# afriesen/rdis

Hardware: AMD Instinct MI355X
Metric: subspace-solver iters/sec (all components), ladybug BA (higher is better)
Workload: dtype f64

## Files before the change

rdis_amd/csrc/minimizer.hpp:

```cpp
#pragma once
#include <hip/hip_runtime.h>
#include <cfloat>
#include <type_traits>
#include <utility>

namespace rdis_hip {

enum : int {
    EXIT_FTOL = 0, EXIT_GTOL = 1, EXIT_GGZERO = 2, EXIT_ITMAX = 3, EXIT_DBRENT_ITMAX = 4,
    EXIT_NAN = 5, EXIT_EMPTY = 6, EXIT_SYNC_TIMEOUT = 7
};
constexpr int STATUS_ROLLED_BACK = 0x100;

enum : int { TR_NONE = 0, TR_F = 1, TR_FD = 2, TR_ITER = 3, TR_START = 4, TR_LINMIN = 5 };

enum : int { REQ_EVAL = 0, REQ_GRAD, REQ_LINE_END, REQ_DONE };
enum : int {
    RF_SLOPE = 1,
    RF_RESTORE = 2,
    RF_LINE = 4,
    RF_PRE_START = 8,
    RF_PRE_UPDATE = 16,
    RF_PRE_BEGIN = 32,
    RF_PRE_LINE_END = 64,
    RF_POST_REDUCE = 128,
    RF_TR_FIRST = 256
};

constexpr int SPEC_MAX = 4;

struct Request {
    int kind;
    int flags;
    int ncand;
    double cand[SPEC_MAX - 1];
    int pre_tag;
    int tr_tag;
    double a, b;
    double pre_a, pre_b, pre_c;
    double tr_a, tr_b, tr_c;
};

__device__ __forceinline__ void opaque(double& v) { asm("" : "+v"(v)); }

struct Predictor {
    enum : int { P_STOP = 0, P_BR_FC, P_DB };
    int ph;
    bool need_first;
    bool known;
    double a, b, x, dx;
    double w, v, dw, dv, d, e;
    double uu;
    double ax, bx, cx;

    __device__ void start(const struct CgdMachine& M, bool swapped);
    __device__ void begin_brent(double ax_, double bx_, double cx_, bool slope_known, double slope) {
        a = (ax_ < cx_ ? ax_ : cx_);
        b = (ax_ > cx_ ? ax_ : cx_);
        x = bx_;
        need_first = !slope_known;
        dx = slope_known ? slope : -1.0;
        ph = P_DB;
        known = false; w = v = x; dw = dv = dx; d = e = 0.0; uu = x;
    }
    __device__ bool next(double& c) {
#pragma clang fp contract(off)
        const double GOLD = 1.618034, TOL = 3.0e-8, ZEPS = DBL_EPSILON * 1.0e-3;
        if (ph == P_BR_FC) {
            cx = bx + GOLD * (bx - ax);
            c = cx;
            if (bx == 0.0) begin_brent(ax, bx, cx, false, 0.0); else ph = P_STOP;
            return true;
        }
        if (ph != P_DB) return false;
        if (need_first) { need_first = false; c = x; return true; }
        const double xm = 0.5 * (a + b);
        const double tol1 = TOL * fabs(x) + ZEPS;
        const double tol2 = 2.0 * tol1;
        if (fabs(x - xm) <= (tol2 - 0.5 * (b - a))) { ph = P_STOP; return false; }
        const double ebis = (dx >= 0.0 ? a - x : b - x);
        const bool near = (uu - x) * (w - x) > 0.0 && fabs(uu - x) < fabs(w - x);
        const bool exact = known && w != x && v != x && v != w && !near;
        double dn = 0.5 * ebis, en = ebis;
        if (exact) {
            const bool big = fabs(e) > tol1;
            const double dflt = 2.0 * (b - a);
            const double q1 = (w - x) * dx / (dx - dw);
            const double q2 = (v - x) * dx / (dx - dv);
            const double d1 = (dw != dx) ? q1 : dflt;
            const double d2 = (dv != dx) ? q2 : dflt;
            const double u1 = x + d1, u2 = x + d2;
            const bool ok1 = (a - u1) * (u1 - b) > 0.0 && dx * d1 <= 0.0;
            const bool ok2 = (a - u2) * (u2 - b) > 0.0 && dx * d2 <= 0.0;
            const double dsel = (ok1 && ok2) ? (fabs(d1) < fabs(d2) ? d1 : d2) : (ok1 ? d1 : d2);
            const bool accept = big && (ok1 || ok2) && (fabs(dsel) <= fabs(0.5 * e));
            const double ut = x + dsel;
            const double dacc = (ut - a < tol2 || b - ut < tol2) ? copysign(tol1, xm - x) : dsel;
            en = accept ? d : ebis;
            dn = accept ? dacc : 0.5 * ebis;
        } else {
            known = false;
        }
        const bool tn = !(fabs(dn) >= tol1);
        const double u = tn ? x + copysign(tol1, dn) : x + dn;
        c = u;
        d = dn; e = en; uu = u;
        if (tn) ph = P_STOP;
        else if (u < x) a = u; else b = u;
// ... 37 lines not shown
    __device__ int status() const { return reason | (rolled_back ? STATUS_ROLLED_BACK : 0); }

    __device__ static Request req(int kind, double a = 0.0, int flags = 0) {
        Request r; r.kind = kind; r.a = a; r.b = 0.0; r.flags = flags;
        r.ncand = 0;
        for (int k = 0; k < SPEC_MAX - 1; ++k) r.cand[k] = 0.0;
        r.pre_tag = TR_NONE; r.pre_a = r.pre_b = r.pre_c = 0.0;
        r.tr_tag = TR_NONE; r.tr_a = r.tr_b = r.tr_c = 0.0;
        return r;
    }
    __device__ Request with_pending(Request r) {
        r.pre_tag = pp_tag; r.pre_a = pp_a; r.pre_b = pp_b; r.pre_c = pp_c;
        pp_tag = TR_NONE;
        return r;
    }
    __device__ static Request traced(Request r, int tag, double ta, double tb, double tc) {
        r.tr_tag = tag; r.tr_a = ta; r.tr_b = tb; r.tr_c = tc;
        return r;
    }
    __device__ Request want_f(double at, bool line = true) { ++nfeval; return req(REQ_EVAL, at, line ? RF_LINE : 0); }
    __device__ Request want_fd(double at, int extra = 0) { ++nfeval; return req(REQ_EVAL, at, RF_SLOPE | RF_LINE | extra); }
    __device__ Request start_line(int pre_ops, double gamma) {
        iter = its;
        ax = 0.0; bx = 1.0;
        fa = fp; sa = 0.0; va = false;
        if (noskip) {
            st = S_BR_FA;
            Request r = want_f(ax);
            r.flags |= pre_ops | RF_PRE_BEGIN;
            r.b = gamma;
            return r;
        }
        ++nfeval;
        pp_tag = TR_F; pp_a = 0.0; pp_b = fp; pp_c = 0.0;
        st = S_BR_FB;
        Request r = with_pending(want_fd(bx, pre_ops | RF_PRE_BEGIN));
        r.b = gamma;
        return r;
    }
    __device__ Request line_done() {
        if (2.0 * fabs(fx - fp) <= ftol * (fabs(fx) + fabs(fp) + 1.0e-18)) {
            st = S_AFTER_LINMIN;
            return traced(req(REQ_LINE_END, x), TR_LINMIN, x, fx, 0.0);
        }
        fret = fx;
        fp = fret;
        ++ngeval;
        st = S_REDUCED;
        Request r = req(REQ_GRAD, x, RF_PRE_LINE_END | RF_POST_REDUCE);
        r.b = fp;
        return traced(r, TR_LINMIN, x, fx, 0.0);
    }

    __device__ __forceinline__ bool hot(double r0, double r1, double& un, int& pre_tag, double& pre_a, double& pre_b,
                                        double& pre_c, Predictor& G) {
#pragma clang fp contract(off)
        const double TOL = 3.0e-8, ZEPS = DBL_EPSILON * 1.0e-3;
        const int DB_ITMAX = 100;
        double a_ = a, b_ = b, x_ = x, w_ = w, v_ = v, fx_ = fx, fw_ = fw, fv_ = fv;
        double dx_ = dx, dw_ = dw, dv_ = dv, d_ = d, e_ = e, uu_ = uu;
        long long nfe_ = nfeval, nge_ = ngeval;
        int ppt_ = pp_tag;
        double ppa_ = pp_a, ppb_ = pp_b, ppc_ = pp_c;
        const bool tiny_ = tiny;
        const int it_ = it;
        if (st != S_DB_EVAL) return false;
        opaque(a_); opaque(b_); opaque(x_); opaque(w_); opaque(v_); opaque(fx_); opaque(fw_); opaque(fv_);
        opaque(dx_); opaque(dw_); opaque(dv_); opaque(d_); opaque(e_); opaque(uu_);
        opaque(ppa_); opaque(ppb_); opaque(ppc_);
        asm("" : "+v"(nfe_), "+v"(nge_), "+v"(ppt_));
        if ((tiny_ && r0 > fx_) || !(it_ + 1 < DB_ITMAX)) return false;
        const double fu = r0, du = r1;
        const bool le = fu <= fx_;
        const bool right = uu_ >= x_, left = uu_ < x_;
        const double a1 = le ? (right ? x_ : a_) : (left ? uu_ : a_);
        const double b1 = le ? (right ? b_ : x_) : (left ? b_ : uu_);
        const bool c1 = !le && (fu <= fw_ || w_ == x_);
        const bool c2 = !le && !c1 && (fu < fv_ || v_ == x_ || v_ == w_);
        const bool vw = le || c1;
        const double v1 = vw ? w_ : (c2 ? uu_ : v_), fv1 = vw ? fw_ : (c2 ? fu : fv_), dv1 = vw ? dw_ : (c2 ? du : dv_);
        const double w1 = le ? x_ : (c1 ? uu_ : w_), fw1 = le ? fx_ : (c1 ? fu : fw_), dw1 = le ? dx_ : (c1 ? du : dw_);
        const double x1 = le ? uu_ : x_, fx1 = le ? fu : fx_, dx1 = le ? du : dx_;
        const double xm = 0.5 * (a1 + b1);
        const double tol1 = TOL * fabs(x1) + ZEPS;
        const double tol2 = 2.0 * tol1;
        if (fabs(x1 - xm) <= (tol2 - 0.5 * (b1 - a1))) return false;
        const bool big = fabs(e_) > tol1;
        const double dflt = 2.0 * (b1 - a1);
        const double q1 = (w1 - x1) * dx1 / (dx1 - dw1);
        const double q2 = (v1 - x1) * dx1 / (dx1 - dv1);
        const double d1 = (dw1 != dx1) ? q1 : dflt;
        const double d2 = (dv1 != dx1) ? q2 : dflt;
        const double u1 = x1 + d1, u2 = x1 + d2;
        const bool ok1 = (a1 - u1) * (u1 - b1) > 0.0 && dx1 * d1 <= 0.0;
        const bool ok2 = (a1 - u2) * (u2 - b1) > 0.0 && dx1 * d2 <= 0.0;
        const double dsel = (ok1 && ok2) ? (fabs(d1) < fabs(d2) ? d1 : d2) : (ok1 ? d1 : d2);
        const bool accept = big && (ok1 || ok2) && (fabs(dsel) <= fabs(0.5 * e_));
        const double ut = x1 + dsel;
        const double dacc = (ut - a1 < tol2 || b1 - ut < tol2) ? copysign(tol1, xm - x1) : dsel;
        const double ebis = (dx1 >= 0.0 ? a1 - x1 : b1 - x1);
        const double enew = accept ? d_ : ebis;
        const double dnew = accept ? dacc : 0.5 * ebis;
        const bool tn = !(fabs(dnew) >= tol1);
        un = tn ? x1 + copysign(tol1, dnew) : x1 + dnew;
        if (fu != fu) saw_nan = true;
        a = a1; b = b1; v = v1; fv = fv1; dv = dv1; w = w1; fw = fw1; dw = dw1; x = x1; fx = fx1; dx = dx1;
        e = enew; d = dnew; tiny = tn; uu = un;
        it = it_ + 1;
        ngeval = nge_ + 1;
        nfeval = nfe_ + 1;
        pp_tag = TR_NONE;
        pre_tag = ppt_; pre_a = ppa_; pre_b = ppb_; pre_c = ppc_;
        G.need_first = false;
        G.a = (!tn && un < x1) ? un : a1;
        G.b = (!tn && !(un < x1)) ? un : b1;
        G.x = x1; G.dx = dx1;
        G.known = true; G.w = w1; G.v = v1; G.dw = dw1; G.dv = dv1; G.d = dnew; G.e = enew; G.uu = un;
        G.ph = tn ? Predictor::P_STOP : Predictor::P_DB;
        return true;
    }

    __device__ Request next(double r0, double r1, double r2) {
#pragma clang fp contract(off)
        const double GOLD = 1.618034, GLIMIT = 100.0, TINY = 1.0e-20;
        const double GTOL = 1.0e-8;
        const double TOL = 3.0e-8;
        const double ZEPS = DBL_EPSILON * 1.0e-3;
        const int DB_ITMAX = 100;
        for (;;) {
            switch (st) {
            case S_BEGIN:
                st = S_FIRST;
                return want_f(0.0, false);
            case S_FIRST:
                finit = r0;
                if (r0 != r0) saw_nan = true;
                ++nfeval;
                fp = finit;
                ++ngeval;
                st = S_GRAD0;
                return traced(req(REQ_GRAD), TR_START, fp, 0.0, 0.0);
            case S_GRAD0:
                its = 0;
                return start_line(RF_PRE_START, 0.0);

            case S_BR_FA:
                fa = r0; if (r0 != r0) saw_nan = true;
                st = S_BR_FB;
                return want_fd(bx);
            case S_BR_FB:
                fb = r0; sb = r1; vb = true; if (r0 != r0) saw_nan = true;
                if (fb > fa) {
                    double t = ax; ax = bx; bx = t; t = fa; fa = fb; fb = t;
                    t = sa; sa = sb; sb = t; const bool tv = va; va = vb; vb = tv;
                }
                cx = bx + GOLD * (bx - ax);
                st = S_BR_FC;
                return want_fd(cx);
            case S_BR_FC:
                fc = r0; sc = r1; vc = true; if (r0 != r0) saw_nan = true;
                st = S_BR_HEAD;
                break;
            case S_BR_HEAD: {
                if (!(fb > fc)) { st = S_DB_START; break; }
                const double r = (bx - ax) * (fb - fc);
                const double q = (bx - cx) * (fb - fa);
                const double qr = q - r;
                u = bx - ((bx - cx) * q - (bx - ax) * r) / (2.0 * copysign(fmax(fabs(qr), TINY), qr));
                const double ulim = bx + GLIMIT * (cx - bx);
                if ((bx - u) * (u - cx) > 0.0) { st = S_BR_CASE1; return want_fd(u); }
                if ((cx - u) * (u - ulim) > 0.0) { st = S_BR_CASE2; return want_fd(u); }
                if ((u - ulim) * (ulim - cx) >= 0.0) u = ulim;
// ... 122 lines not shown
                if (test < GTOL) { reason = EXIT_GTOL; st = S_FINISH; nx = finish_request(); }
                else if (gg == 0.0) { reason = EXIT_GGZERO; st = S_FINISH; nx = finish_request(); }
                else if (its + 1 >= maxiters) { reason = EXIT_ITMAX; st = S_FINISH; nx = finish_request(); }
                else { ++its; nx = start_line(RF_PRE_UPDATE, dgg / gg); nx.flags |= RF_TR_FIRST; }
                return traced(nx, TR_ITER, test, gg, dgg);
            }

            case S_FINISH: {
                Request nx = finish_request();
                return nx;
            }
            case S_ROLLED:
                fret = r0;
                st = S_DONE;
                return req(REQ_DONE);
            default:
                return req(REQ_DONE);
            }
        }
    }

    __device__ Request finish_request() {
        if (saw_nan) { reason = EXIT_NAN; fret = DBL_MAX; }
        if (fret > finit || saw_nan) {
            rolled_back = true;
            st = S_ROLLED;
            Request r = want_f(0.0, false);
            r.flags |= RF_RESTORE;
            return r;
        }
        st = S_DONE;
        return req(REQ_DONE);
    }
};

__device__ inline void Predictor::start(const CgdMachine& M, bool swapped) {
#pragma clang fp contract(off)
    ph = P_STOP; need_first = false; known = false;
    a = b = x = dx = 0.0; ax = bx = cx = 0.0;
    w = v = dw = dv = d = e = uu = 0.0;
    switch (M.st) {
    case CgdMachine::S_BR_FB:
        if (swapped) { ax = M.bx; bx = M.ax; ph = P_BR_FC; }
        else { ax = M.ax; bx = M.bx; ph = P_BR_FC; }
        break;
    case CgdMachine::S_BR_FC:
        begin_brent(M.ax, M.bx, M.cx, M.vb, M.sb);
        break;
    case CgdMachine::S_DB_FIRST:
        a = M.a; b = M.b; x = M.x; dx = -1.0; ph = P_DB;
        w = v = x; dw = dv = dx; uu = x;
        break;
    case CgdMachine::S_DB_EVAL:
        if (M.tiny) break;
        a = M.a; b = M.b; x = M.x; dx = M.dx; ph = P_DB;
        if (M.uu < x) a = M.uu; else b = M.uu;
        known = true; w = M.w; v = M.v; dw = M.dw; dv = M.dv; d = M.d; e = M.e; uu = M.uu;
        break;
    default: break;
    }
}

__device__ __forceinline__ void step_machine(CgdMachine* __restrict__ M, Request* __restrict__ out, double r0, double r1, double r2,
                                             bool writer) {
    double un, pa, pb, pc;
    int ptag;
    Predictor G;
    if (M->hot(r0, r1, un, ptag, pa, pb, pc, G)) {
        if (writer) {
            out->kind = REQ_EVAL; out->flags = RF_SLOPE | RF_LINE; out->ncand = 0;
            out->pre_tag = ptag; out->tr_tag = TR_NONE; out->a = un;
            if (ptag != TR_NONE) { out->pre_a = pa; out->pre_b = pb; out->pre_c = pc; }
        }
        return;
    }
    const Request nq = M->next(r0, r1, r2);
    if (writer) {
        out->kind = nq.kind; out->flags = nq.flags; out->ncand = 0;
        out->pre_tag = nq.pre_tag; out->tr_tag = nq.tr_tag; out->a = nq.a; out->b = nq.b;
        if (nq.pre_tag != TR_NONE) { out->pre_a = nq.pre_a; out->pre_b = nq.pre_b; out->pre_c = nq.pre_c; }
        if (nq.tr_tag != TR_NONE) { out->tr_a = nq.tr_a; out->tr_b = nq.tr_b; out->tr_c = nq.tr_c; }
    }
}

__device__ __forceinline__ double uniform(double v) {
    const long long b = __double_as_longlong(v);
    const unsigned lo = __builtin_amdgcn_readfirstlane((unsigned)b);
    const unsigned hi = __builtin_amdgcn_readfirstlane((unsigned)((unsigned long long)b >> 32));
    return __longlong_as_double((long long)(((unsigned long long)hi << 32) | lo));
}

template <class Env>
__device__ __forceinline__ double uni(double v) {
    if constexpr (Env::UNIFORM) return uniform(v); else return v;
}
template <class Env>
__device__ __forceinline__ int uni(int v) {
    if constexpr (Env::UNIFORM) return __builtin_amdgcn_readfirstlane(v); else return v;
}

template <int N>
__device__ __forceinline__ double pick(const double (&v)[N], int j) {
    double r = v[0];
#pragma unroll
    for (int k = 1; k < N; ++k) r = (j == k) ? v[k] : r;
    return r;
}
__device__ __forceinline__ bool same_bits(double a, double b) { return __double_as_longlong(a) == __double_as_longlong(b); }

template <class E, class = void> struct EnvNoSkip { static constexpr bool value = false; };
// ... 178 lines not shown
```

rdis_amd/csrc/solver_pipe.hpp:

```cpp
#pragma once
#include "solver_coop.hpp"

namespace rdis_hip {

constexpr int PIPE_NBUF = 32;
constexpr int PIPE_DEPTH = 3;
constexpr int PIPE_ENT = 512;
constexpr int PIPE_MAILS = 4;
constexpr int PIPE_THREADS = 256;
constexpr int PIPE_CTRL = 2;
constexpr int PIPE_LANES = PIPE_THREADS - 64 * PIPE_CTRL;
constexpr int PIPE_QUIT = 0x7FFFFFFF;
static_assert(PIPE_NBUF >= 5 * PIPE_DEPTH + 4 && (PIPE_NBUF & (PIPE_NBUF - 1)) == 0, "ring too short for the run-ahead");

struct PipeState {
    alignas(32) unsigned long long granule[2][PIPE_NBUF][PIPE_ENT][2];
    unsigned int abort_flag;
    unsigned int pad[15];
};
static_assert(sizeof(PipeState) <= sizeof(CoopState), "PipeState must fit the exchange state the host allocates");

struct alignas(16) PipeMail {
    int kind, flags;
    int e;
    int pad0;
    double a, b;
    double g_a, g_b, g_x, g_dx, g_ax, g_bx, g_cx;
    int g_need_first, g_known;
    double g_w, g_v, g_dw, g_dv, g_d, g_e, g_uu;
    int g_ph, pad1;
};
static_assert(sizeof(PipeMail) == 160, "mail layout");
constexpr int PIPE_RES = 4;
static_assert(PIPE_RES > PIPE_DEPTH, "result ring");
constexpr int PIPE_RECS = 8;
struct PipeShared {
    PipeMail mail[PIPE_MAILS];
    alignas(8) int seq;
    int verified;
    int pred_seq;
    int rec_slot[PIPE_RECS];
    double rec_val[PIPE_RECS];
    int cmd, cmd_delay;
    int res_slot[PIPE_RES];
    double res[PIPE_RES][3];
    int bar_done;
    int pub[PIPE_LANES / 64];
    int dead;
    int status, rolled_back, iter;
    long long nfeval, ngeval;
    double fret, finit;
};
typedef __attribute__((address_space(3))) int lds_i32;
typedef __attribute__((address_space(3))) double lds_f64;
__device__ __forceinline__ int lds_int(const int& x) { return *(const volatile lds_i32*)&x; }
__device__ __forceinline__ void lds_set(int& x, int v) { *(volatile lds_i32*)&x = v; }
typedef __attribute__((address_space(3))) long long lds_i64;
__device__ __forceinline__ long long lds_int_pair(const int& x) { return *(const volatile lds_i64*)&x; }
__device__ __forceinline__ double lds_f64_get(const double& x) { return *(const volatile lds_f64*)&x; }
__device__ __forceinline__ void lds_f64_set(double& x, double v) { *(volatile lds_f64*)&x = v; }

struct PipeSync {
    PipeState* st;
    int tid, nwg, wg, nw;
    int poll_delay;
    int e;
    int rearmed;
    bool dead;
#ifdef RDIS_COOP_TIMING
    long long tm[COOP_TM];
#endif
    __device__ void tick(int slot, long long dt) {
#ifdef RDIS_COOP_TIMING
        tm[slot] += dt;
#endif
    }
    __device__ gu64* gran(int ex, int k, int w) const { return (gu64*)&st->granule[k >> 1][ex & (PIPE_NBUF - 1)][w][k & 1]; }
    __device__ u64x2 load_pair(int ex, int k, int w) const {
        u64x2 r;
        const gu64* p = gran(ex, k, w);
        asm volatile("global_load_dwordx4 %0, %1, off sc1" : "=v"(r) : "v"(p) : "memory");
        return r;
    }
    __device__ void store_pair(int ex, int k, int w, unsigned long long a, unsigned long long b) const {
        u64x2 t; t.x = a; t.y = b;
        gu64* p = gran(ex, k, w);
        asm volatile("global_store_dwordx4 %0, %1, off sc1" : : "v"(p), "v"(t) : "memory");
    }

    template <int N, int NMAX>
    __device__ void publish(int ex, double (&v)[N], int* pub) {
#pragma unroll
        for (int k = 0; k < N; ++k) v[k] = k < N - NMAX ? wave_sum(v[k]) : wave_max(v[k]);
        asm volatile("s_waitcnt vmcnt(0)" ::: "memory");
        if ((tid & 63) == 0) {
            const int ent = wg * nw + (tid >> 6) - PIPE_CTRL;
#pragma unroll
            for (int k = 0; k + 1 < N; k += 2) store_pair(ex, k, ent, GridSync::bits_of(v[k]), GridSync::bits_of(v[k + 1]));
            if constexpr (N & 1) GridSync::publish(gran(ex, N - 1, ent), v[N - 1]);
            lds_set(pub[(tid >> 6) - PIPE_CTRL], ex);
        }
    }

    template <int N, int NMAX>
// ... 297 lines not shown
        { const double gn = -wv.xi; const double hn = gn + gam * wv.h; wv.g = gn; wv.h = hn; wv.xi = hn; }
    }
    __device__ void write_back(const VarState& V, bool restore, bool writer) {
        if (V.li >= 0 && writer) {
            const double xf = clampd(restore ? V.xinit : V.p, V.lo, V.hi);
            P.x[L.free_vid[f0 + V.li]] = xf;
            L.xout[f0 + V.li] = xf;
        }
    }
};

__device__ __forceinline__ int pipe_slot_owner(int i) {
    return (i == 0 || i == 2 || i == 3 || i == 18 || (i >= 9 && i <= 11) || i == 30 || i == 31) ? 2 : (i == 1 || (i >= 4 && i <= 6) || (i >= 26 && i <= 29)) ? 1 : 0;
}

__device__ __forceinline__ void pipe_post(PipeShared& S, int seq, int kind, int flags, int e, double a, double b, bool writer) {
    if (writer) {
        PipeMail* m = &S.mail[seq & (PIPE_MAILS - 1)];
        m->kind = kind; m->flags = flags; m->e = e; m->pad0 = 0; m->a = a; m->b = b;
        asm volatile("" ::: "memory");
        lds_set(S.seq, seq);
    }
}
__device__ __forceinline__ void pipe_post_predictor(PipeShared& S, int seq, const Predictor& G, bool writer) {
    if (writer) {
        PipeMail* m = &S.mail[seq & (PIPE_MAILS - 1)];
        m->g_ph = G.ph; m->g_need_first = G.need_first ? 1 : 0; m->g_known = G.known ? 1 : 0; m->pad1 = 0;
        m->g_a = G.a; m->g_b = G.b; m->g_x = G.x; m->g_dx = G.dx; m->g_ax = G.ax; m->g_bx = G.bx; m->g_cx = G.cx;
        m->g_w = G.w; m->g_v = G.v; m->g_dw = G.dw; m->g_dv = G.dv; m->g_d = G.d; m->g_e = G.e; m->g_uu = G.uu;
        asm volatile("" ::: "memory");
        lds_set(S.pred_seq, seq);
    }
}
__device__ __forceinline__ void pipe_command(PipeShared& S, int ex, int n, int delay, bool writer) {
    if (writer) { lds_set(S.cmd_delay, delay); lds_set(S.cmd, (ex << 2) | n); }
}
template <int N>
__device__ __forceinline__ void pipe_result(PipeShared& S, int ex, double (&v)[N], bool& dead) {
    while (lds_int(S.res_slot[ex & (PIPE_RES - 1)]) != ex) __builtin_amdgcn_s_sleep(1);
    asm volatile("" ::: "memory");
#pragma unroll
    for (int k = 0; k < N; ++k) v[k] = uniform(lds_f64_get(S.res[ex & (PIPE_RES - 1)][k]));
    if (lds_int(S.dead) != 0) dead = true;
}
__device__ __forceinline__ void pipe_ctrl_barrier(PipeSync& X, PipeShared& S, bool writer) {
    double z[1];
    pipe_command(S, X.e, 1, X.poll_delay, writer);
    pipe_result(S, X.e, z, X.dead);
    if (writer) lds_set(S.bar_done, X.e);
    ++X.e;
}

__device__ __forceinline__ void pipe_stepper(PipeEnv& E, PipeShared& S, int maxiters, double ftol) {
    CgdMachine M;
    M.init(maxiters, ftol);
    int e_last = 0;
    bool chain_live = false;
    int next_free = 0;
    bool swapped = true;
    double r0 = 0.0, r1 = 0.0, r2 = 0.0;
    int seq = 0;
    const bool writer = E.tid == 0;
    for (;;) {
        const long long ts0 = coop_clock();
        bool guessed = false;
        double gval = 0.0;
        int ahead_slot = -1;
        double ahead0 = 0.0, ahead1 = 0.0;
        if (chain_live) {
            const int z = e_last + 1;
            int rec = lds_int(S.rec_slot[z & (PIPE_RECS - 1)]);
            ahead_slot = lds_int(S.res_slot[z & (PIPE_RES - 1)]);
            ahead0 = lds_f64_get(S.res[z & (PIPE_RES - 1)][0]);
            ahead1 = lds_f64_get(S.res[z & (PIPE_RES - 1)][1]);
            while ((rec >> 1) != z) { __builtin_amdgcn_s_sleep(1); rec = lds_int(S.rec_slot[z & (PIPE_RECS - 1)]); }
            guessed = (rec & 1) != 0;
            gval = uniform(lds_f64_get(S.rec_val[z & (PIPE_RECS - 1)]));
        }
        asm volatile("; PIPE_STEP_BEGIN");
        Request nq;
        Predictor G;
        G.ph = Predictor::P_STOP; G.need_first = false; G.known = false; G.a = G.b = G.x = G.dx = 0.0; G.ax = G.bx = G.cx = 0.0;
        G.w = G.v = G.dw = G.dv = G.d = G.e = G.uu = 0.0;
        bool was_hot;
        {
            double un, pa, pb, pc;
            int ptag;
            Predictor unused;
            was_hot = M.hot(r0, r1, un, ptag, pa, pb, pc, unused);
            if (was_hot) {
                nq = CgdMachine::req(REQ_EVAL, un, RF_SLOPE | RF_LINE);
                nq.pre_tag = ptag; nq.pre_a = pa; nq.pre_b = pb; nq.pre_c = pc;
            } else {
                nq = M.next(r0, r1, r2);
                if (M.st == CgdMachine::S_BR_FC) swapped = M.ax == 1.0;
            }
        }
        if (E.X.dead) {
            nq = CgdMachine::req(REQ_DONE);
            M.reason = EXIT_SYNC_TIMEOUT; M.rolled_back = true; M.fret = M.finit;
        }
        const bool slope = nq.kind == REQ_EVAL && (nq.flags & RF_SLOPE) != 0;
        const bool hit = slope && nq.flags == (RF_SLOPE | RF_LINE) && guessed && same_bits(nq.a, gval);
        int e;
        if (hit) {
            e = e_last + 1;
            if (writer) lds_set(S.verified, e);
        } else {
            e = next_free;
            pipe_post(S, ++seq, nq.kind, nq.flags, e, nq.a, nq.b, writer);
            if (slope) {
                if (E.A.speculate) G.start(M, swapped);
                pipe_post_predictor(S, seq, G, writer);
            }
        }
        if (E.tr != nullptr) {
            if ((nq.flags & RF_TR_FIRST) && nq.tr_tag != TR_NONE) E.trace(nq.tr_tag, nq.tr_a, nq.tr_b, nq.tr_c);
            if (nq.pre_tag != TR_NONE) E.trace(nq.pre_tag, nq.pre_a, nq.pre_b, nq.pre_c);
            if (!(nq.flags & RF_TR_FIRST) && nq.tr_tag != TR_NONE) E.trace(nq.tr_tag, nq.tr_a, nq.tr_b, nq.tr_c);
        }
        asm volatile("; PIPE_STEP_END");
        const long long ts1 = coop_clock();
        E.X.tick(8, ts1 - ts0);
        if (nq.kind == REQ_DONE) break;
        E.X.e = e;
        chain_live = false;
        [[maybe_unused]] const int tkind = nq.kind == REQ_GRAD ? 2 : !slope ? 0 : (nq.flags & (RF_PRE_START | RF_PRE_UPDATE)) ? 3 : 1;
        switch (nq.kind) {
        case REQ_EVAL:
            if (nq.flags & RF_PRE_START) pipe_ctrl_barrier(E.X, S, writer);
            if (slope) {
                if (!hit) pipe_command(S, E.X.e, 2, E.X.poll_delay, writer);
                double v[2];
                const long long tw0 = coop_clock();
                if (hit && __builtin_amdgcn_readfirstlane(ahead_slot) == E.X.e) {
                    v[0] = uniform(ahead0); v[1] = uniform(ahead1);
                    if (lds_int(S.dead) != 0) E.X.dead = true;
                } else {
                    pipe_result(S, E.X.e, v, E.X.dead);
                }
                if (hit) { E.X.tick(20, coop_clock() - tw0); E.X.tick(16, 1); }
                else { E.X.tick(21, coop_clock() - tw0); E.X.tick(17, 1); }
                r0 = v[0]; r1 = v[1];
                e_last = E.X.e;
                chain_live = true;
                next_free = e_last + PIPE_DEPTH + 1;
                E.trace(TR_FD, nq.a, r0, r1);
            } else {
                double v[1];
                pipe_command(S, E.X.e, 1, E.X.poll_delay, writer);
                pipe_result(S, E.X.e, v, E.X.dead);
                r0 = v[0];
                next_free = E.X.e + 1;
                if (nq.flags & RF_LINE) E.trace(TR_F, nq.a, r0, 0.0);
            }
            break;
        case REQ_GRAD:
            pipe_ctrl_barrier(E.X, S, writer);
            if (nq.flags & RF_POST_REDUCE) {
                double v[3];
                pipe_command(S, E.X.e, 3, E.X.poll_delay, writer);
                pipe_result(S, E.X.e, v, E.X.dead);
                ++E.X.e;
                r1 = v[0]; r2 = v[1]; r0 = v[2];
            }
            next_free = E.X.e;
            break;
        default:
            break;
        }
        if (tkind == 0) { E.X.tick(12, coop_clock() - ts1); E.X.tick(22, 1); }
        else if (tkind == 1) { E.X.tick(13, coop_clock() - ts1); E.X.tick(23, 1); }
        else if (tkind == 2) { E.X.tick(14, coop_clock() - ts1); E.X.tick(24, 1); }
        else { E.X.tick(15, coop_clock() - ts1); E.X.tick(25, 1); }
    }
    if (writer) {
        lds_set(S.cmd, PIPE_QUIT);
        S.status = M.status(); S.rolled_back = M.rolled_back ? 1 : 0; S.iter = M.iter;
        S.nfeval = M.nfeval; S.ngeval = M.ngeval; S.fret = M.fret; S.finit = M.finit;
    }
}

__device__ __forceinline__ void pipe_collector(PipeSync& X, PipeShared& S) {
    int mine = -1;
    int next = -1;
    const bool writer = (X.tid & 63) == 0;
    for (;;) {
        const int c = lds_int(S.cmd);
        int ex, n;
        if (c != mine) {
            if (c == PIPE_QUIT) break;
            mine = c;
            ex = c >> 2; n = c & 3;
        } else if (next >= 0) {
            ex = next; n = 2;
        } else {
            __builtin_amdgcn_s_sleep(1);
            continue;
        }
        next = -1;
        const int delay = lds_int(S.cmd_delay);
        double v[3] = {0.0, 0.0, 0.0};
        bool got;
        const long long t0 = coop_clock();
        if (n == 2) { double w[2]; got = X.sweep<2, 0>(ex, w, delay, S.cmd, mine, S.pub); v[0] = w[0]; v[1] = w[1]; }
        else if (n == 3) { got = X.sweep<3, 1>(ex, v, delay, S.cmd, mine, S.pub); }
        else { double w[1]; got = X.sweep<1, 0>(ex, w, delay, S.cmd, mine, S.pub); v[0] = w[0]; }
        if (!got) { X.tick(4, 1); continue; }
        X.tick(1, coop_clock() - t0);
        if (writer) {
            if (X.dead) lds_set(S.dead, 1);
            double* r = S.res[ex & (PIPE_RES - 1)];
            lds_f64_set(r[0], v[0]); lds_f64_set(r[1], v[1]); lds_f64_set(r[2], v[2]);
            lds_set(S.res_slot[ex & (PIPE_RES - 1)], ex);
        }
        asm volatile("s_waitcnt vmcnt(0)" ::: "memory");
        X.rearm_behind(ex);
        if (n == 2 && !X.dead) {
            const int z = ex + 1;
            for (;;) {
                const int rec = lds_int(S.rec_slot[z & (PIPE_RECS - 1)]);
                if ((rec >> 1) == z) { if (rec & 1) next = z; break; }
                if (lds_int(S.cmd) != mine) break;
                __builtin_amdgcn_s_sleep(1);
            }
        }
    }
}

__device__ __forceinline__ void pipe_record(PipeShared& S, int z, bool valid, double val, bool writer) {
    if (writer) {
        lds_f64_set(S.rec_val[z & (PIPE_RECS - 1)], val);
// ... 48 lines not shown
                for (;;) {
                    const long long sv = lds_int_pair(S.seq);
                    if (!cvalid || (int)sv != seen) break;
                    const int ver = (int)(sv >> 32);
                    if (cz > (ver > e0 ? ver : e0) + PIPE_DEPTH) { __builtin_amdgcn_s_sleep(1); continue; }
                    const double ca = cval;
                    const int z = cz;
                    cvalid = G.next(cval);
                    cz = z + 1;
                    pipe_record(S, cz, cvalid, cval, recorder);
                    double v[2];
                    const long long te0 = coop_clock();
                    E.eval_line<true>(ca, v[0], v[1]);
                    const long long te1 = coop_clock();
                    E.X.publish<2, 0>(z, v, S.pub);
                    E.X.tick(0, te1 - te0); E.X.tick(2, coop_clock() - te1); E.X.tick(11, 1);
                }
            } else {
                if (flags & RF_RESTORE) E.load_base(E.L.xstart + E.f0);
                double v[1], dummy;
                E.eval_line<false>((flags & RF_RESTORE) ? 0.0 : qa, v[0], dummy);
                E.X.publish<1, 0>(E.X.e, v, S.pub);
            }
        } else if (kind == REQ_GRAD) {
            if (flags & RF_PRE_LINE_END) E.line_end(qa);
            E.gradient_to_xi();
            if (flags & RF_POST_REDUCE) E.cg_reduce_publish(uniform(m->b));
        } else if (kind == REQ_LINE_END) {
            E.line_end(qa);
        }
    }
}

template <int THREADS>
__device__ __forceinline__ void pipe_solve(const ProblemView& P, const PlanView& L, const CoopArgs& A, int nwg, int wg,
                                           int maxiters, double ftol) {
    static_assert(THREADS == PIPE_THREADS, "stepper + collector + two lane waves");
    __shared__ PipeShared S;
    [[maybe_unused]] const long long tk0 = coop_clock();
    const int comp = A.comp;
    const int f0 = L.free_ptr[comp], c0 = L.fac_ptr[comp];
    const int n = L.free_ptr[comp + 1] - f0, m = L.fac_ptr[comp + 1] - c0;
    const int tid = (int)threadIdx.x;
    const int gt = tid < 64 * PIPE_CTRL ? -1 : wg * PIPE_LANES + tid - 64 * PIPE_CTRL;

    PipeEnv E{P, L, A, S, n, m, f0, c0, gt, tid,
              PipeSync{(PipeState*)A.st, tid, nwg, wg, PIPE_LANES / 64, A.poll_delay, 0, -1, false
#ifdef RDIS_COOP_TIMING
                       , {}
#endif
              },
              L.trace ? L.trace + 4ll * L.trace_cap * comp : nullptr, 0, 0,
              gt >= 0 && gt < m, 0, {}, {}, {}, {}, {}, 0.0, 0.0, {}, {}};
    if (E.has_fac) {
        E.fid = L.fac_id[c0 + gt];
        const double2 o = P.obs[E.fid];
        E.ox = o.x; E.oy = o.y;
        const int* sp = L.slot_pos + L.slot_base[c0 + gt];
#pragma unroll
        for (int k = 0; k < 12; ++k) E.gpos[k] = sp[k];
    }
    if (tid == 0) { S.seq = 0; S.pred_seq = 0; S.cmd = -1; S.cmd_delay = 0; S.bar_done = -1; S.dead = 0; S.verified = -1; }
    if (tid < PIPE_RECS) S.rec_slot[tid] = -1;
    if (tid < PIPE_RES) S.res_slot[tid] = -1;
    if (tid < PIPE_LANES / 64) S.pub[tid] = -1;
    E.init_vectors();
    __syncthreads();
    if (tid < 64) pipe_stepper(E, S, maxiters, ftol);
    else if (tid < 128) pipe_collector(E.X, S);
    else pipe_lanes(E, S);
    __syncthreads();
    const bool restore = S.rolled_back != 0;
    E.write_back(E.lv, restore, true);
    E.write_back(E.wv, restore, (tid & 63) == 0);
    if (wg == 0 && tid == 0) {
        L.fret[comp] = S.fret; L.delta[comp] = S.fret - S.finit; L.iters[comp] = S.iter;
        L.status[comp] = S.status; L.nfeval[comp] = S.nfeval; L.ngeval[comp] = S.ngeval;
        if (L.trace_n) L.trace_n[comp] = E.trn;
    }
#ifdef RDIS_COOP_TIMING
    if (wg == 0 && (tid & 63) == 0 && tid < 192 && A.timing) {
        if (tid == 0) E.X.tm[7] = coop_clock() - tk0;
        for (int i = 0; i < COOP_TM; ++i) if (pipe_slot_owner(i) == (tid >> 6)) A.timing[i] = E.X.tm[i];
    }
#endif
}

template <int THREADS>
__global__ void __launch_bounds__(THREADS)
cgd_pipe_kernel(ProblemView P, PlanView L, const CoopGroup* __restrict__ groups, const int* __restrict__ wg_group,
                int maxiters, double ftol) {
    const CoopGroup G = groups[wg_group[blockIdx.x]];
    pipe_solve<THREADS>(P, L, G.a, G.nwg, (int)blockIdx.x - G.wg0, maxiters, ftol);
}
template <int THREADS>
__global__ void __launch_bounds__(THREADS)
cgd_pipe_single_kernel(ProblemView P, PlanView L, CoopArgs A, int maxiters, double ftol) {
    pipe_solve<THREADS>(P, L, A, (int)gridDim.x, (int)blockIdx.x, maxiters, ftol);
}

__global__ void __launch_bounds__(256) pipe_arm_kernel(const CoopGroup* __restrict__ groups) {
    const CoopGroup G = groups[blockIdx.x / PIPE_NBUF];
    const int b = blockIdx.x % PIPE_NBUF;
    PipeState* st = (PipeState*)G.a.st;
    const int entries = G.nwg * (PIPE_LANES / 64);
    for (int t = threadIdx.x; t < COOP_KP * entries; t += blockDim.x) {
        const int k = t % COOP_KP, e = t / COOP_KP;
        st->granule[k >> 1][b][e][k & 1] = ~0ull;
    }
    if (b == 0 && threadIdx.x == 0) st->abort_flag = 0u;
}

inline int launch_pipe(hipStream_t stream, int kind, const ProblemView& P, const PlanView& V, const CoopGroup& first,
                       const CoopGroup* groups, const int* wg_group, int ngroups, int total_wg, int maxiters, double ftol) {
    if (kind != KIND_BA) return (int)hipErrorNotSupported;
    pipe_arm_kernel<<<ngroups * PIPE_NBUF, 256, 0, stream>>>(groups);
    hipError_t e0 = hipGetLastError();
    if (e0 != hipSuccess) return (int)e0;
    ProblemView p = P;
    PlanView v = V;
    int mi = maxiters;
    double ft = ftol;
    if (ngroups == 1) {
        CoopArgs a = first.a;
        void* args[] = {&p, &v, &a, &mi, &ft};
        return (int)hipLaunchCooperativeKernel((const void*)cgd_pipe_single_kernel<PIPE_THREADS>, dim3(total_wg), dim3(PIPE_THREADS), args, 0, stream);
    }
// ... 17 lines not shown
```

Baseline: 9876.

## Split Brent hot step into precomputed pre/post phases with a dedicated stepper loop

The Brent line-search hot step is split into hot_pre, which precomputes both branch outcomes (left/right bracket, tolerances, secant quotients) while the function/derivative evaluation is in flight, and hot_post, a branch-free select once the result arrives. The stepper now runs a tight inner loop for S_DB_EVAL. The CgdMachine moves into LDS, and only the writer lane mutates it. Lane setup and write-back move into the lane waves, which spin on a fin flag so they can overlap with the stepper. The aim is to cut serial latency on the stepper's critical path, at the cost of more complex control flow and a risk of subtle numerical divergence or race issues.

```diff
diff --git a/rdis_amd/csrc/minimizer.hpp b/rdis_amd/csrc/minimizer.hpp
--- a/rdis_amd/csrc/minimizer.hpp
+++ b/rdis_amd/csrc/minimizer.hpp
@@ -41,7 +41,26 @@
     double tr_a, tr_b, tr_c;
 };
 
-__device__ __forceinline__ void opaque(double& v) { asm("" : "+v"(v)); }
+__host__ __device__ __forceinline__ void opaque(double& v) {
+#ifdef __HIP_DEVICE_COMPILE__
+    asm("" : "+v"(v));
+#else
+    (void)v;
+#endif
+}
+
+struct BrentHot {
+    double a, b, x, w, v, fx, fw, fv, dx, dw, dv, d, e, uu;
+    long long nfeval, ngeval;
+    int it;
+    bool tiny, saw_nan;
+};
+struct HotPre {
+    double aL, bL, xmL, tol1L, tol2L, dfltL;
+    double aG, bG, xmG, tol1G, tol2G, dfltG;
+    double qw, qv;
+    bool convL, bigL, convG, bigG, stop;
+};
 
 struct Predictor {
     enum : int { P_STOP = 0, P_BR_FC, P_DB };
@@ -54,6 +73,15 @@
     double ax, bx, cx;
 
     __device__ void start(const struct CgdMachine& M, bool swapped);
+    __device__ void start_eval(const BrentHot& s) {
+        ph = P_STOP; need_first = false; known = false;
+        a = b = x = dx = 0.0; ax = bx = cx = 0.0;
+        w = v = dw = dv = d = e = uu = 0.0;
+        if (s.tiny) return;
+        a = s.a; b = s.b; x = s.x; dx = s.dx; ph = P_DB;
+        if (s.uu < x) a = s.uu; else b = s.uu;
+        known = true; w = s.w; v = s.v; dw = s.dw; dv = s.dv; d = s.d; e = s.e; uu = s.uu;
+    }
     __device__ void begin_brent(double ax_, double bx_, double cx_, bool slope_known, double slope) {
         a = (ax_ < cx_ ? ax_ : cx_);
         b = (ax_ > cx_ ? ax_ : cx_);
@@ -197,7 +225,7 @@
         return traced(r, TR_LINMIN, x, fx, 0.0);
     }
 
-    __device__ __forceinline__ bool hot(double r0, double r1, double& un, int& pre_tag, double& pre_a, double& pre_b,
+    __host__ __device__ __forceinline__ bool hot(double r0, double r1, double& un, int& pre_tag, double& pre_a, double& pre_b,
                                         double& pre_c, Predictor& G) {
 #pragma clang fp contract(off)
         const double TOL = 3.0e-8, ZEPS = DBL_EPSILON * 1.0e-3;
@@ -213,7 +241,9 @@
         opaque(a_); opaque(b_); opaque(x_); opaque(w_); opaque(v_); opaque(fx_); opaque(fw_); opaque(fv_);
         opaque(dx_); opaque(dw_); opaque(dv_); opaque(d_); opaque(e_); opaque(uu_);
         opaque(ppa_); opaque(ppb_); opaque(ppc_);
+#ifdef __HIP_DEVICE_COMPILE__
         asm("" : "+v"(nfe_), "+v"(nge_), "+v"(ppt_));
+#endif
         if ((tiny_ && r0 > fx_) || !(it_ + 1 < DB_ITMAX)) return false;
         const double fu = r0, du = r1;
         const bool le = fu <= fx_;
@@ -263,6 +293,92 @@
         G.known = true; G.w = w1; G.v = v1; G.dw = dw1; G.dv = dv1; G.d = dnew; G.e = enew; G.uu = un;
         G.ph = tn ? Predictor::P_STOP : Predictor::P_DB;
         return true;
+    }
+
+    __host__ __device__ __forceinline__ BrentHot brent() const {
+        BrentHot s;
+        s.a = a; s.b = b; s.x = x; s.w = w; s.v = v; s.fx = fx; s.fw = fw; s.fv = fv;
+        s.dx = dx; s.dw = dw; s.dv = dv; s.d = d; s.e = e; s.uu = uu;
+        s.nfeval = nfeval; s.ngeval = ngeval; s.it = it; s.tiny = tiny; s.saw_nan = saw_nan;
+        return s;
+    }
+    __host__ __device__ __forceinline__ void set_brent(const BrentHot& s) {
+        a = s.a; b = s.b; x = s.x; w = s.w; v = s.v; fx = s.fx; fw = s.fw; fv = s.fv;
+        dx = s.dx; dw = s.dw; dv = s.dv; d = s.d; e = s.e; uu = s.uu;
+        nfeval = s.nfeval; ngeval = s.ngeval; it = s.it; tiny = s.tiny; saw_nan = s.saw_nan;
+    }
+    __host__ __device__ static __forceinline__ void hot_pre(const BrentHot& s0, HotPre& P) {
+#pragma clang fp contract(off)
+        BrentHot s = s0;
+        opaque(s.a); opaque(s.b); opaque(s.x); opaque(s.w); opaque(s.v); opaque(s.dx); opaque(s.dw); opaque(s.dv); opaque(s.e); opaque(s.uu);
+        const double TOL = 3.0e-8, ZEPS = DBL_EPSILON * 1.0e-3;
+        const int DB_ITMAX = 100;
+        const bool right = s.uu >= s.x, left = s.uu < s.x;
+        P.stop = !(s.it + 1 < DB_ITMAX);
+        P.aL = right ? s.x : s.a;
+        P.bL = right ? s.b : s.x;
+        P.xmL = 0.5 * (P.aL + P.bL);
+        P.tol1L = TOL * fabs(s.uu) + ZEPS;
+        P.tol2L = 2.0 * P.tol1L;
+        P.convL = fabs(s.uu - P.xmL) <= (P.tol2L - 0.5 * (P.bL - P.aL));
+        P.bigL = fabs(s.e) > P.tol1L;
+        P.dfltL = 2.0 * (P.bL - P.aL);
+        P.aG = left ? s.uu : s.a;
+        P.bG = left ? s.b : s.uu;
+        P.xmG = 0.5 * (P.aG + P.bG);
+        P.tol1G = TOL * fabs(s.x) + ZEPS;
+        P.tol2G = 2.0 * P.tol1G;
+        P.convG = fabs(s.x - P.xmG) <= (P.tol2G - 0.5 * (P.bG - P.aG));
+        P.bigG = fabs(s.e) > P.tol1G;
+        P.dfltG = 2.0 * (P.bG - P.aG);
+        P.qw = (s.w - s.x) * s.dx / (s.dx - s.dw);
+        P.qv = (s.v - s.x) * s.dx / (s.dx - s.dv);
+    }
+    __host__ __device__ static __forceinline__ bool hot_post(const BrentHot& s0, const HotPre& P0, double fu, double du, BrentHot& n,
+                                                             double& un) {
+#pragma clang fp contract(off)
+        BrentHot s = s0;
+        HotPre P = P0;
+        opaque(s.a); opaque(s.b); opaque(s.x); opaque(s.w); opaque(s.v); opaque(s.fx); opaque(s.fw); opaque(s.fv);
+        opaque(s.dx); opaque(s.dw); opaque(s.dv); opaque(s.d); opaque(s.e); opaque(s.uu);
+        opaque(P.aL); opaque(P.bL); opaque(P.xmL); opaque(P.tol1L); opaque(P.tol2L); opaque(P.dfltL);
+        opaque(P.aG); opaque(P.bG); opaque(P.xmG); opaque(P.tol1G); opaque(P.tol2G); opaque(P.dfltG); opaque(P.qw); opaque(P.qv);
+        const bool le = fu <= s.fx;
+        const bool c1 = !le && (fu <= s.fw || s.w == s.x);
+        const bool c2 = !le && !c1 && (fu < s.fv || s.v == s.x || s.v == s.w);
+        const bool vw = le || c1;
+        const double v1 = vw ? s.w : (c2 ? s.uu : s.v), fv1 = vw ? s.fw : (c2 ? fu : s.fv), dv1 = vw ? s.dw : (c2 ? du : s.dv);
+        const double w1 = le ? s.x : (c1 ? s.uu : s.w), fw1 = le ? s.fx : (c1 ? fu : s.fw), dw1 = le ? s.dx : (c1 ? du : s.dw);
+        const double x1 = le ? s.uu : s.x, fx1 = le ? fu : s.fx, dx1 = le ? du : s.dx;
+        const double a1 = le ? P.aL : P.aG, b1 = le ? P.bL : P.bG, xm = le ? P.xmL : P.xmG;
+        const double tol1 = le ? P.tol1L : P.tol1G, tol2 = le ? P.tol2L : P.tol2G, dflt = le ? P.dfltL : P.dfltG;
+        const bool conv = le ? P.convL : P.convG, big = le ? P.bigL : P.bigG;
+        const double qa = (le ? s.x - s.uu : s.uu - s.x) * (le ? du : s.dx) / (le ? du - s.dx : s.dx - du);
+        const double qb = (s.w - s.uu) * du / (du - s.dw);
+        const double q1 = vw ? qa : P.qw;
+        const double q2 = le ? qb : (c1 ? P.qw : (c2 ? qa : P.qv));
+        const double d1 = (dw1 != dx1) ? q1 : dflt;
+        const double d2 = (dv1 != dx1) ? q2 : dflt;
+        const double u1 = x1 + d1, u2 = x1 + d2;
+        const bool ok1 = (a1 - u1) * (u1 - b1) > 0.0 && dx1 * d1 <= 0.0;
+        const bool ok2 = (a1 - u2) * (u2 - b1) > 0.0 && dx1 * d2 <= 0.0;
+        const double dsel = (ok1 && ok2) ? (fabs(d1) < fabs(d2) ? d1 : d2) : (ok1 ? d1 : d2);
+        const bool accept = big && (ok1 || ok2) && (fabs(dsel) <= fabs(0.5 * s.e));
+        const double ut = x1 + dsel;
+        const double dacc = (ut - a1 < tol2 || b1 - ut < tol2) ? copysign(tol1, xm - x1) : dsel;
+        const double ebis = (dx1 >= 0.0 ? a1 - x1 : b1 - x1);
+        const double enew = accept ? s.d : ebis;
+        const double dnew = accept ? dacc : 0.5 * ebis;
+        const bool tn = !(fabs(dnew) >= tol1);
+        un = tn ? x1 + copysign(tol1, dnew) : x1 + dnew;
+        const bool taken = !((s.tiny && fu > s.fx) || P.stop || conv);
+        const bool nan = s.saw_nan || fu != fu;
+        const long long nfe = s.nfeval + 1, nge = s.ngeval + 1;
+        const int it1 = s.it + 1;
+        n.a = a1; n.b = b1; n.v = v1; n.fv = fv1; n.dv = dv1; n.w = w1; n.fw = fw1; n.dw = dw1; n.x = x1; n.fx = fx1; n.dx = dx1;
+        n.e = enew; n.d = dnew; n.tiny = tn; n.uu = un;
+        n.it = it1; n.ngeval = nge; n.nfeval = nfe; n.saw_nan = nan;
+        return taken;
     }
 
     __device__ Request next(double r0, double r1, double r2) {
@@ -491,10 +607,7 @@
         w = v = x; dw = dv = dx; uu = x;
         break;
     case CgdMachine::S_DB_EVAL:
-        if (M.tiny) break;
-        a = M.a; b = M.b; x = M.x; dx = M.dx; ph = P_DB;
-        if (M.uu < x) a = M.uu; else b = M.uu;
-        known = true; w = M.w; v = M.v; dw = M.dw; dv = M.dv; d = M.d; e = M.e; uu = M.uu;
+        start_eval(M.brent());
         break;
     default: break;
     }
diff --git a/rdis_amd/csrc/solver_pipe.hpp b/rdis_amd/csrc/solver_pipe.hpp
--- a/rdis_amd/csrc/solver_pipe.hpp
+++ b/rdis_amd/csrc/solver_pipe.hpp
@@ -48,8 +48,10 @@
     int pub[PIPE_LANES / 64];
     int dead;
     int status, rolled_back, iter;
+    int fin;
     long long nfeval, ngeval;
     double fret, finit;
+    CgdMachine mach;
 };
 typedef __attribute__((address_space(3))) int lds_i32;
 typedef __attribute__((address_space(3))) double lds_f64;
@@ -453,21 +455,21 @@
 }
 
 __device__ __forceinline__ void pipe_stepper(PipeEnv& E, PipeShared& S, int maxiters, double ftol) {
-    CgdMachine M;
-    M.init(maxiters, ftol);
+    CgdMachine& M = S.mach;
+    const bool writer = E.tid == 0;
+    if (writer) M.init(maxiters, ftol);
     int e_last = 0;
     bool chain_live = false;
     int next_free = 0;
     bool swapped = true;
     double r0 = 0.0, r1 = 0.0, r2 = 0.0;
     int seq = 0;
-    const bool writer = E.tid == 0;
-    for (;;) {
-        const long long ts0 = coop_clock();
-        bool guessed = false;
-        double gval = 0.0;
-        int ahead_slot = -1;
-        double ahead0 = 0.0, ahead1 = 0.0;
+    bool guessed = false;
+    double gval = 0.0;
+    int ahead_slot = -1;
+    double ahead0 = 0.0, ahead1 = 0.0;
+    auto read_chain = [&]() {
+        guessed = false; gval = 0.0; ahead_slot = -1; ahead0 = ahead1 = 0.0;
         if (chain_live) {
             const int z = e_last + 1;
             int rec = lds_int(S.rec_slot[z & (PIPE_RECS - 1)]);
@@ -478,74 +480,120 @@
             guessed = (rec & 1) != 0;
             gval = uniform(lds_f64_get(S.rec_val[z & (PIPE_RECS - 1)]));
         }
-        asm volatile("; PIPE_STEP_BEGIN");
+    };
+    auto await_fd = [&](int e, bool hit) {
+        double v[2];
+        const long long tw0 = coop_clock();
+        if (hit && __builtin_amdgcn_readfirstlane(ahead_slot) == e) {
+            v[0] = uniform(ahead0); v[1] = uniform(ahead1);
+            if (lds_int(S.dead) != 0) E.X.dead = true;
+        } else {
+            pipe_result(S, e, v, E.X.dead);
+        }
+        if (hit) { E.X.tick(20, coop_clock() - tw0); E.X.tick(16, 1); }
+        else { E.X.tick(21, coop_clock() - tw0); E.X.tick(17, 1); }
+        r0 = v[0]; r1 = v[1];
+        e_last = e;
+        chain_live = true;
+        next_free = e_last + PIPE_DEPTH + 1;
+    };
+    for (;;) {
+        long long ts0 = coop_clock();
+        read_chain();
+        bool stepped = false;
+        if (__builtin_amdgcn_readfirstlane(lds_int(M.st)) == CgdMachine::S_DB_EVAL) {
+            BrentHot s = M.brent();
+            opaque(s.a); opaque(s.b); opaque(s.x); opaque(s.w); opaque(s.v); opaque(s.fx); opaque(s.fw); opaque(s.fv);
+            opaque(s.dx); opaque(s.dw); opaque(s.dv); opaque(s.d); opaque(s.e); opaque(s.uu);
+            HotPre P;
+            CgdMachine::hot_pre(s, P);
+            for (;;) {
+                asm volatile("; PIPE_STEP_BEGIN");
+                BrentHot n;
+                double un;
+                const bool take = CgdMachine::hot_post(s, P, r0, r1, n, un);
+                if (__builtin_amdgcn_readfirstlane(take ? 1 : 0) == 0) break;
+                s = n;
+                if (E.X.dead) { stepped = true; break; }
+                const bool hit = __builtin_amdgcn_readfirstlane((guessed && same_bits(un, gval)) ? 1 : 0) != 0;
+                int e;
+                if (hit) {
+                    e = e_last + 1;
+                    if (writer) lds_set(S.verified, e);
+                } else {
+                    e = next_free;
+                    pipe_post(S, ++seq, REQ_EVAL, RF_SLOPE | RF_LINE, e, un, 0.0, writer);
+                    Predictor G;
+                    G.ph = Predictor::P_STOP; G.need_first = false; G.known = false; G.a = G.b = G.x = G.dx = 0.0; G.ax = G.bx = G.cx = 0.0;
+                    G.w = G.v = G.dw = G.dv = G.d = G.e = G.uu = 0.0;
+                    if (E.A.speculate) G.start_eval(s);
+                    pipe_post_predictor(S, seq, G, writer);
+                }
+                asm volatile("; PIPE_STEP_END");
+                const long long ts1 = coop_clock();
+                E.X.tick(8, ts1 - ts0);
+                E.X.e = e;
+                if (!hit) pipe_command(S, e, 2, E.X.poll_delay, writer);
+                CgdMachine::hot_pre(s, P);
+                await_fd(e, hit);
+                E.trace(TR_FD, un, r0, r1);
+                E.X.tick(13, coop_clock() - ts1); E.X.tick(23, 1);
+                ts0 = coop_clock();
+                read_chain();
+            }
+            if (writer) M.set_brent(s);
+        }
+        asm volatile("; PIPE_GENERIC_BEGIN");
         Request nq;
-        Predictor G;
-        G.ph = Predictor::P_STOP; G.need_first = false; G.known = false; G.a = G.b = G.x = G.dx = 0.0; G.ax = G.bx = G.cx = 0.0;
-        G.w = G.v = G.dw = G.dv = G.d = G.e = G.uu = 0.0;
-        bool was_hot;
-        {
-            double un, pa, pb, pc;
-            int ptag;
-            Predictor unused;
-            was_hot = M.hot(r0, r1, un, ptag, pa, pb, pc, unused);
-            if (was_hot) {
-                nq = CgdMachine::req(REQ_EVAL, un, RF_SLOPE | RF_LINE);
-                nq.pre_tag = ptag; nq.pre_a = pa; nq.pre_b = pb; nq.pre_c = pc;
-            } else {
+        if (writer) {
+            if (!stepped) {
                 nq = M.next(r0, r1, r2);
                 if (M.st == CgdMachine::S_BR_FC) swapped = M.ax == 1.0;
-            }
-        }
-        if (E.X.dead) {
-            nq = CgdMachine::req(REQ_DONE);
-            M.reason = EXIT_SYNC_TIMEOUT; M.rolled_back = true; M.fret = M.finit;
-        }
-        const bool slope = nq.kind == REQ_EVAL && (nq.flags & RF_SLOPE) != 0;
-        const bool hit = slope && nq.flags == (RF_SLOPE | RF_LINE) && guessed && same_bits(nq.a, gval);
+            } else {
+                nq = CgdMachine::req(REQ_DONE);
+            }
+            if (E.X.dead) {
+                nq = CgdMachine::req(REQ_DONE);
+                M.reason = EXIT_SYNC_TIMEOUT; M.rolled_back = true; M.fret = M.finit;
+            }
+        }
+        const int kind = __builtin_amdgcn_readfirstlane(nq.kind);
+        const int flags = __builtin_amdgcn_readfirstlane(nq.flags);
+        const bool slope = kind == REQ_EVAL && (flags & RF_SLOPE) != 0;
+        const bool hit = __builtin_amdgcn_readfirstlane((slope && flags == (RF_SLOPE | RF_LINE) && guessed && same_bits(nq.a, gval)) ? 1 : 0) != 0;
         int e;
         if (hit) {
             e = e_last + 1;
             if (writer) lds_set(S.verified, e);
         } else {
             e = next_free;
-            pipe_post(S, ++seq, nq.kind, nq.flags, e, nq.a, nq.b, writer);
-            if (slope) {
+            pipe_post(S, ++seq, kind, flags, e, nq.a, nq.b, writer);
+            if (slope && writer) {
+                Predictor G;
+                G.ph = Predictor::P_STOP; G.need_first = false; G.known = false; G.a = G.b = G.x = G.dx = 0.0; G.ax = G.bx = G.cx = 0.0;
+                G.w = G.v = G.dw = G.dv = G.d = G.e = G.uu = 0.0;
                 if (E.A.speculate) G.start(M, swapped);
                 pipe_post_predictor(S, seq, G, writer);
             }
         }
         if (E.tr != nullptr) {
-            if ((nq.flags & RF_TR_FIRST) && nq.tr_tag != TR_NONE) E.trace(nq.tr_tag, nq.tr_a, nq.tr_b, nq.tr_c);
+            if ((flags & RF_TR_FIRST) && nq.tr_tag != TR_NONE) E.trace(nq.tr_tag, nq.tr_a, nq.tr_b, nq.tr_c);
             if (nq.pre_tag != TR_NONE) E.trace(nq.pre_tag, nq.pre_a, nq.pre_b, nq.pre_c);
-            if (!(nq.flags & RF_TR_FIRST) && nq.tr_tag != TR_NONE) E.trace(nq.tr_tag, nq.tr_a, nq.tr_b, nq.tr_c);
-        }
-        asm volatile("; PIPE_STEP_END");
+            if (!(flags & RF_TR_FIRST) && nq.tr_tag != TR_NONE) E.trace(nq.tr_tag, nq.tr_a, nq.tr_b, nq.tr_c);
+        }
+        asm volatile("; PIPE_GENERIC_END");
         const long long ts1 = coop_clock();
         E.X.tick(8, ts1 - ts0);
-        if (nq.kind == REQ_DONE) break;
+        if (kind == REQ_DONE) break;
         E.X.e = e;
         chain_live = false;
-        [[maybe_unused]] const int tkind = nq.kind == REQ_GRAD ? 2 : !slope ? 0 : (nq.flags & (RF_PRE_START | RF_PRE_UPDATE)) ? 3 : 1;
-        switch (nq.kind) {
+        [[maybe_unused]] const int tkind = kind == REQ_GRAD ? 2 : !slope ? 0 : (flags & (RF_PRE_START | RF_PRE_UPDATE)) ? 3 : 1;
+        switch (kind) {
         case REQ_EVAL:
-            if (nq.flags & RF_PRE_START) pipe_ctrl_barrier(E.X, S, writer);
+            if (flags & RF_PRE_START) pipe_ctrl_barrier(E.X, S, writer);
             if (slope) {
                 if (!hit) pipe_command(S, E.X.e, 2, E.X.poll_delay, writer);
-                double v[2];
-                const long long tw0 = coop_clock();
-                if (hit && __builtin_amdgcn_readfirstlane(ahead_slot) == E.X.e) {
-                    v[0] = uniform(ahead0); v[1] = uniform(ahead1);
-                    if (lds_int(S.dead) != 0) E.X.dead = true;
-                } else {
-                    pipe_result(S, E.X.e, v, E.X.dead);
-                }
-                if (hit) { E.X.tick(20, coop_clock() - tw0); E.X.tick(16, 1); }
-                else { E.X.tick(21, coop_clock() - tw0); E.X.tick(17, 1); }
-                r0 = v[0]; r1 = v[1];
-                e_last = E.X.e;
-                chain_live = true;
-                next_free = e_last + PIPE_DEPTH + 1;
+                await_fd(E.X.e, hit);
                 E.trace(TR_FD, nq.a, r0, r1);
             } else {
                 double v[1];
@@ -553,12 +601,12 @@
                 pipe_result(S, E.X.e, v, E.X.dead);
                 r0 = v[0];
                 next_free = E.X.e + 1;
-                if (nq.flags & RF_LINE) E.trace(TR_F, nq.a, r0, 0.0);
+                if (flags & RF_LINE) E.trace(TR_F, nq.a, r0, 0.0);
             }
             break;
         case REQ_GRAD:
             pipe_ctrl_barrier(E.X, S, writer);
-            if (nq.flags & RF_POST_REDUCE) {
+            if (flags & RF_POST_REDUCE) {
                 double v[3];
                 pipe_command(S, E.X.e, 3, E.X.poll_delay, writer);
                 pipe_result(S, E.X.e, v, E.X.dead);
@@ -579,6 +627,8 @@
         lds_set(S.cmd, PIPE_QUIT);
         S.status = M.status(); S.rolled_back = M.rolled_back ? 1 : 0; S.iter = M.iter;
         S.nfeval = M.nfeval; S.ngeval = M.ngeval; S.fret = M.fret; S.finit = M.finit;
+        asm volatile("" ::: "memory");
+        lds_set(S.fin, 1);
     }
 }
 
@@ -733,27 +783,31 @@
               },
               L.trace ? L.trace + 4ll * L.trace_cap * comp : nullptr, 0, 0,
               gt >= 0 && gt < m, 0, {}, {}, {}, {}, {}, 0.0, 0.0, {}, {}};
-    if (E.has_fac) {
-        E.fid = L.fac_id[c0 + gt];
-        const double2 o = P.obs[E.fid];
-        E.ox = o.x; E.oy = o.y;
-        const int* sp = L.slot_pos + L.slot_base[c0 + gt];
-#pragma unroll
-        for (int k = 0; k < 12; ++k) E.gpos[k] = sp[k];
-    }
-    if (tid == 0) { S.seq = 0; S.pred_seq = 0; S.cmd = -1; S.cmd_delay = 0; S.bar_done = -1; S.dead = 0; S.verified = -1; }
+    if (tid == 0) { S.seq = 0; S.pred_seq = 0; S.cmd = -1; S.cmd_delay = 0; S.bar_done = -1; S.dead = 0; S.verified = -1; S.fin = 0; }
     if (tid < PIPE_RECS) S.rec_slot[tid] = -1;
     if (tid < PIPE_RES) S.res_slot[tid] = -1;
     if (tid < PIPE_LANES / 64) S.pub[tid] = -1;
-    E.init_vectors();
     __syncthreads();
-    if (tid < 64) pipe_stepper(E, S, maxiters, ftol);
-    else if (tid < 128) pipe_collector(E.X, S);
-    else pipe_lanes(E, S);
+    const int role = __builtin_amdgcn_readfirstlane(tid >> 6);
+    if (role == 0) pipe_stepper(E, S, maxiters, ftol);
+    else if (role == 1) pipe_collector(E.X, S);
+    else {
+        if (E.has_fac) {
+            E.fid = L.fac_id[c0 + gt];
+            const double2 o = P.obs[E.fid];
+            E.ox = o.x; E.oy = o.y;
+            const int* sp = L.slot_pos + L.slot_base[c0 + gt];
+#pragma unroll
+            for (int k = 0; k < 12; ++k) E.gpos[k] = sp[k];
+        }
+        E.init_vectors();
+        pipe_lanes(E, S);
+        while (lds_int(S.fin) == 0) __builtin_amdgcn_s_sleep(1);
+        const bool restore = S.rolled_back != 0;
+        E.write_back(E.lv, restore, true);
+        E.write_back(E.wv, restore, (tid & 63) == 0);
+    }
     __syncthreads();
-    const bool restore = S.rolled_back != 0;
-    E.write_back(E.lv, restore, true);
-    E.write_back(E.wv, restore, (tid & 63) == 0);
     if (wg == 0 && tid == 0) {
         L.fret[comp] = S.fret; L.delta[comp] = S.fret - S.finit; L.iters[comp] = S.iter;
         L.status[comp] = S.status; L.nfeval[comp] = S.nfeval; L.ngeval[comp] = S.ngeval;
```

After: 10230, median of 6. +3.6%, better.
